# mlvlab/BLiM

Measured on AMD Instinct MI355X. Metric: candidate-pairs/sec (7B, 96+32 tok), higher is better.
Workload: dtype f16; 1 GPU; SYN v2t-VTG re-rank: Qwen2-7B dims (28 layers), seeded synthetic weights, 96 video + 32 text tokens per pair, top-16 text candidates per video query, 55 queries (880 pairs, 32560 packed tokens, 28160 label rows) per step per GPU; prefix_reuse=True, vtg_compensated=none, parallelism=query rows sharded over 1 GPU(s); RCCL all-gather of score rows at the end

## Files before the change

### blim_amd/csrc/attention.hip

```cpp
#include "attention.hpp"

#include <stdlib.h>

#include <type_traits>

#define HD 128
#define KT 32
#define QB 32

typedef __attribute__((ext_vector_type(4))) short s16x4;

template <int MAXC, bool SPLIT> struct attn_bound { static constexpr int value = MAXC <= (SPLIT ? 8 : 4) ? 512 : MAXC <= (SPLIT ? 16 : 8) ? 256 : 64; };
template <bool USE_TR, int MAXC, int DT, bool SPLIT = false, bool OUT_LO = SPLIT, bool PC = false>
__global__ __launch_bounds__((attn_bound<MAXC, SPLIT>::value)) void attn_kernel(const typename std::conditional<PC, AttnPcParams, AttnParams>::type p) {
    __shared__ __attribute__((aligned(16))) bf16_t k_lds[(SPLIT ? 2 : 1) * KT * HD];
    __shared__ __attribute__((aligned(16))) bf16_t v_lds[(SPLIT ? 2 : 1) * KT * HD];
    __shared__ uint32_t vis_lds[KT / 4];

    const int tid = threadIdx.x, nthreads = blockDim.x;
    const int lane = tid & 63;
    const int wave = tid >> 6;
    const int G = p.num_heads / p.num_kv_heads;
    const int ngrp = (int)gridDim.y / p.num_kv_heads;
    const int kh = blockIdx.y / ngrp, hg = blockIdx.y - kh * ngrp;
// ... 253 lines not shown
            if (hf == 0) {
                const int rl = (int)(tok & 255);
                p.out_mx[(int64_t)head * p.mx_stride + (tok >> 8) * 256 + ((rl >> 7) * 16 + (rl & 15)) * 8 + ((rl >> 4) & 7)] = (uint8_t)(e + 127);
            }
        }
        return;
    }
    if (q0 + qi < slen) {
        const float inv = l_run > 0.f ? 1.0f / l_run : 0.f;
        bf16_t* orow = p.out + (int64_t)(sstart + q0 + qi) * p.ldo + head * HD;
        if (p.lse_out && hf == 0) p.lse_out[(int64_t)(sstart + q0 + qi) * p.num_heads + head] = l_run > 0.f ? m_run * p.scale + __logf(l_run) : 1.0e30f;
#pragma unroll
        for (int db = 0; db < 4; ++db)
#pragma unroll
            for (int g = 0; g < 4; ++g) {
                const int d = 32 * db + 8 * g + 4 * hf;
                const float x0 = o[db][4 * g] * inv, x1 = o[db][4 * g + 1] * inv, x2 = o[db][4 * g + 2] * inv, x3 = o[db][4 * g + 3] * inv;
                *(uint2*)(orow + d) = make_uint2(pack2<DT>(x0, x1), pack2<DT>(x2, x3));
                if constexpr (OUT_LO)
                    *(uint2*)(orow + p.out_lo_off + d) = make_uint2(pack2<DT>(x0 - from16<DT>(to16<DT>(x0)), x1 - from16<DT>(to16<DT>(x1))),
                                                                    pack2<DT>(x2 - from16<DT>(to16<DT>(x2)), x3 - from16<DT>(to16<DT>(x3))));
            }
    }
}

static bool stages_tile(int maxc, const dim3& block, bool split) {
    if (maxc * (int)block.x >= (split ? 2048 : 1024)) return true;
    blim_set_error("attention: %d threads x %d staging chunks do not cover a tile's %d", (int)block.x, maxc, split ? 2048 : 1024);
    return false;
}

static int launch_attention_pc(const AttnPcParams& p, int G, hipStream_t stream) {
    const dim3 grid(p.n_blocks, p.num_kv_heads), block(64 * G);
    static const int g_split = getenv("BLIM_ATTN_HEAD_GROUPS") ? atoi(getenv("BLIM_ATTN_HEAD_GROUPS")) : 2;
#define ATTN_PC(MC, SP, OL, GRID, BLOCK)                                                                                           \
    do {                                                                                                                       \
        if (!stages_tile(MC, BLOCK, SP)) return BLIM_ERR_ARG;                                                                  \
        if (p.dtype == DT_F16) hipLaunchKernelGGL((attn_kernel<true, MC, DT_F16, SP, OL, true>), GRID, BLOCK, 0, stream, p);      \
        else hipLaunchKernelGGL((attn_kernel<true, MC, DT_BF16, SP, OL, true>), GRID, BLOCK, 0, stream, p);                   \
    } while (0)
    if (p.v_lo_off != 0) {
        if (p.out_lo_off) { if (G >= 7) ATTN_PC(5, true, true, grid, block); else ATTN_PC(4, true, true, grid, dim3(512)); }
        else { if (G >= 7) ATTN_PC(5, true, false, grid, block); else ATTN_PC(4, true, false, grid, dim3(512)); }
    } else if (p.out_lo_off != 0) {
        if (G >= 7 && g_split > 1) ATTN_PC(4, false, true, dim3(p.n_blocks, p.num_kv_heads * 2), dim3(64 * ((G + 1) / 2)));
        else if (G >= 5 && g_split > 1) ATTN_PC(8, false, true, dim3(p.n_blocks, p.num_kv_heads * 2), dim3(64 * ((G + 1) / 2)));
// ... 6 lines not shown
        else if (G >= 4) ATTN_PC(4, false, false, grid, block);
        else if (G >= 2) ATTN_PC(8, false, false, grid, block);
        else ATTN_PC(16, false, false, grid, block);
    }
#undef ATTN_PC
    hipError_t e = hipGetLastError();
    if (e != hipSuccess) { blim_set_error("attention launch failed: %s", hipGetErrorString(e)); return BLIM_ERR_HIP; }
    return BLIM_OK;
}

int launch_attention_cached(const AttnPcParams& p, hipStream_t stream) {
    ARG_CHECK(p.qkv && p.out && p.key_visible && p.seq_start && p.seq_len && p.pfx_start && p.pfx_len && p.blk_seq && p.blk_q0);
    ARG_CHECK(p.n_blocks > 0 && p.num_kv_heads > 0 && p.num_heads % p.num_kv_heads == 0);
    ARG_CHECK(p.ldq % 8 == 0 && p.ldo % 4 == 0);
    ARG_CHECK(p.pfx_cache && p.pfx_slot && p.pc_n_slots > 0 && p.pc_max_len > 0 && p.pc_ld % 8 == 0 && p.pc_lo_off % 8 == 0 && p.pc_slot_stride % 8 == 0 && p.pc_lo_off >= 0);
    ARG_CHECK((p.dtype == DT_F16 || p.dtype == DT_BF16) && p.v_lo_off >= 0 && p.out_lo_off >= 0 && p.v_lo_off % 8 == 0 && p.out_lo_off % 4 == 0);
    if (p.out8 || p.lse_out) { blim_set_error("attention: the prefix-cache forms write a 16-bit output and no lse"); return BLIM_ERR_ARG; }
    if (p.v_lo_off != 0 && p.pc_lo_off == 0) { blim_set_error("attention: a compensated call needs a prefix cache that holds lo parts"); return BLIM_ERR_ARG; }
    const int G = p.num_heads / p.num_kv_heads;
    if (G > 8) { blim_set_error("attention: %d query heads per kv head > 8 unsupported", G); return BLIM_ERR_ARG; }
    return launch_attention_pc(p, G, stream);
}

int launch_attention(const AttnParams& p, int use_tr_read, hipStream_t stream) {
    ARG_CHECK(p.qkv && p.out && p.key_visible && p.seq_start && p.seq_len && p.pfx_start && p.pfx_len && p.blk_seq && p.blk_q0);
    ARG_CHECK(p.n_blocks > 0 && p.num_kv_heads > 0 && p.num_heads % p.num_kv_heads == 0);
    ARG_CHECK(p.ldq % 8 == 0 && p.ldo % 4 == 0);
    const int G = p.num_heads / p.num_kv_heads;
    if (G > 8) { blim_set_error("attention: %d query heads per kv head > 8 unsupported", G); return BLIM_ERR_ARG; }
    const dim3 grid(p.n_blocks, p.num_kv_heads), block(64 * G);
    if (p.v_lo_off != 0 || p.out_lo_off != 0)
        ARG_CHECK((p.dtype == DT_F16 || p.dtype == DT_BF16) && p.v_lo_off >= 0 && p.out_lo_off >= 0 && p.v_lo_off % 8 == 0 && p.out_lo_off % 4 == 0 && !p.out8);
    if (p.v_lo_off != 0) {
#define ATTN_SPLIT(MC, BLOCK)                                                                                                       \
        do {                                                                                                                      \
            if (!stages_tile(MC, BLOCK, true)) return BLIM_ERR_ARG;                                                               \
            if (p.out_lo_off) {                                                                                                   \
                if (p.dtype == DT_F16) hipLaunchKernelGGL((attn_kernel<true, MC, DT_F16, true>), grid, BLOCK, 0, stream, p);       \
                else hipLaunchKernelGGL((attn_kernel<true, MC, DT_BF16, true>), grid, BLOCK, 0, stream, p);                    \
            } else {                                                                                                              \
                if (p.dtype == DT_F16) hipLaunchKernelGGL((attn_kernel<true, MC, DT_F16, true, false>), grid, BLOCK, 0, stream, p); \
                else hipLaunchKernelGGL((attn_kernel<true, MC, DT_BF16, true, false>), grid, BLOCK, 0, stream, p);              \
            }                                                                                                                     \
        } while (0)
        if (G >= 7) ATTN_SPLIT(5, block);
        else ATTN_SPLIT(4, dim3(512));
#undef ATTN_SPLIT
        hipError_t e2 = hipGetLastError();
        if (e2 != hipSuccess) { blim_set_error("attention launch failed: %s", hipGetErrorString(e2)); return BLIM_ERR_HIP; }
        return BLIM_OK;
// ... 2 lines not shown
    if (p.out_lo_off != 0) {
#define ATTN_LO(MC, GRID, BLOCK)                                                                                                   \
        do {                                                                                                                     \
            if (!stages_tile(MC, BLOCK, false)) return BLIM_ERR_ARG;                                                             \
            if (p.dtype == DT_F16) hipLaunchKernelGGL((attn_kernel<true, MC, DT_F16, false, true>), GRID, BLOCK, 0, stream, p);   \
            else hipLaunchKernelGGL((attn_kernel<true, MC, DT_BF16, false, true>), GRID, BLOCK, 0, stream, p);                \
        } while (0)
        if (G >= 7 && g_split > 1) ATTN_LO(4, dim3(p.n_blocks, p.num_kv_heads * 2), dim3(64 * ((G + 1) / 2)));
        else if (G >= 5 && g_split > 1) ATTN_LO(8, dim3(p.n_blocks, p.num_kv_heads * 2), dim3(64 * ((G + 1) / 2)));
        else if (G >= 4) ATTN_LO(4, grid, block);
        else if (G >= 2) ATTN_LO(8, grid, block);
        else ATTN_LO(16, grid, block);
#undef ATTN_LO
        hipError_t e3 = hipGetLastError();
        if (e3 != hipSuccess) { blim_set_error("attention launch failed: %s", hipGetErrorString(e3)); return BLIM_ERR_HIP; }
        return BLIM_OK;
    }
#define ATTN_LAUNCH(TR, MC)                                                                             \
    do {                                                                                            \
        if (!stages_tile(MC, block, false)) return BLIM_ERR_ARG;                                    \
        if (p.dtype == DT_F16) hipLaunchKernelGGL((attn_kernel<TR, MC, DT_F16>), grid, block, 0, stream, p); \
        else hipLaunchKernelGGL((attn_kernel<TR, MC, DT_BF16>), grid, block, 0, stream, p);                \
    } while (0)
    if (G >= 5 && g_split > 1 && use_tr_read && !p.out8) {
        const int hpg = (G + 1) / 2;
        const dim3 grid2(p.n_blocks, p.num_kv_heads * 2), block2(64 * hpg);
        if (!stages_tile(hpg >= 4 ? 4 : 8, block2, false)) return BLIM_ERR_ARG;
        if (hpg >= 4) {
            if (p.dtype == DT_F16) hipLaunchKernelGGL((attn_kernel<true, 4, DT_F16>), grid2, block2, 0, stream, p);
            else hipLaunchKernelGGL((attn_kernel<true, 4, DT_BF16>), grid2, block2, 0, stream, p);
        } else {
            if (p.dtype == DT_F16) hipLaunchKernelGGL((attn_kernel<true, 8, DT_F16>), grid2, block2, 0, stream, p);
            else hipLaunchKernelGGL((attn_kernel<true, 8, DT_BF16>), grid2, block2, 0, stream, p);
        }
    } else if (G >= 4) { if (use_tr_read) ATTN_LAUNCH(true, 4); else ATTN_LAUNCH(false, 4); }
    else if (G >= 2) { if (use_tr_read) ATTN_LAUNCH(true, 8); else ATTN_LAUNCH(false, 8); }
    else { if (use_tr_read) ATTN_LAUNCH(true, 16); else ATTN_LAUNCH(false, 16); }
#undef ATTN_LAUNCH
    hipError_t e = hipGetLastError();
    if (e != hipSuccess) { blim_set_error("attention launch failed: %s", hipGetErrorString(e)); return BLIM_ERR_HIP; }
    return BLIM_OK;
}
```

### blim_amd/csrc/attention.hpp

```cpp
#pragma once
#include "common.hpp"

struct AttnParams {
    int dtype;
    const bf16_t* qkv;
    int64_t ldq;
    int num_heads, num_kv_heads;
    const uint8_t* key_visible;
    const int32_t* seq_start;
    const int32_t* seq_len;
    const int32_t* pfx_start;
    const int32_t* pfx_len;
    const int32_t* blk_seq;
    const int32_t* blk_q0;
    const int32_t* own_start;
    int n_blocks;
    bf16_t* out;
    int64_t ldo;
    float scale;
    int64_t v_lo_off, out_lo_off;
    uint8_t* out8;
    int64_t ldo8;
    uint8_t* out_mx;
    int64_t mx_stride;
    float* lse_out;
};

int launch_attention(const AttnParams& p, int use_tr_read, hipStream_t stream);

struct AttnPcParams : AttnParams {
    const bf16_t* pfx_cache;
    const int32_t* pfx_slot;
    int64_t pc_slot_stride, pc_ld, pc_lo_off;
    int pc_n_slots, pc_max_len;
};
int launch_attention_cached(const AttnPcParams& p, hipStream_t stream);
```

### blim_amd/csrc/engine.hip

```cpp
#include <math.h>
#include <stdarg.h>
#include <stddef.h>
#include <stdio.h>
#include <stdlib.h>
#include <string.h>

#include <algorithm>
#include <map>
#include <string>
#include <vector>

#include "engine.hpp"

static thread_local char g_err[1024] = "";
void blim_set_error(const char* fmt, ...) {
    va_list ap;
    va_start(ap, fmt);
    vsnprintf(g_err, sizeof(g_err), fmt, ap);
    va_end(ap);
}
extern "C" const char* blim_last_error(void) { return g_err; }
extern "C" int blim_abi_version(void) { return BLIM_ABI_VERSION; }

static const char* kTimeClassNames[TC_COUNT] = {"gemm_qkv_rope", "attention", "gemm_o_resid", "gemm_gateup_swiglu", "gemm_down_resid",
// ... 837 lines not shown
            const blim_prefix_cache* pc = e->pc_fill;
            const int kvh = 2 * c.num_kv_heads * 128;
            TRY(launch_kv_capture(qkv, (int64_t)pf * e->qkv_n, (int64_t)c.num_heads * 128, (cA && pc->comp) ? e->qkv_n : 0, kvh, e->pc_cap_row, T,
                                  pc->kv + (int64_t)li * pc->max_len * pc->kv_w, pc->slot_stride, pc->kv_w, kvh, pc->max_len, pc->n_slots, s));
        }
        {
            SpanGuard g(e, s, TC_ATTN, 0);
            AttnParams a;
            a.dtype = c.compute_dtype;
            a.qkv = qkv; a.ldq = (int64_t)pf * e->qkv_n; a.num_heads = c.num_heads; a.num_kv_heads = c.num_kv_heads;
            a.key_visible = b->key_visible; a.seq_start = b->seq_start; a.seq_len = b->seq_len; a.pfx_start = b->pfx_start; a.pfx_len = b->pfx_len;
            a.blk_seq = b->blk_seq; a.blk_q0 = b->blk_q0; a.own_start = b->own_start; a.n_blocks = b->n_blocks; a.out = attn; a.ldo = (int64_t)pf * Hq; a.scale = 0.08838834764831845f;
            a.v_lo_off = cA ? e->qkv_n : 0; a.out_lo_off = cO ? Hq : 0;
            a.out8 = nullptr; a.ldo8 = 0; a.out_mx = nullptr; a.mx_stride = 0; a.lse_out = nullptr;
            if (o8 && e->f8_fuse) { a.out8 = a8; a.ldo8 = H; a.out_mx = (uint8_t*)e->attn_mx.p; a.mx_stride = Tp; }
            if (e->pc_read) {
                const blim_prefix_cache* pc = e->pc_read;
                AttnPcParams pa;
                static_cast<AttnParams&>(pa) = a;
                pa.pfx_cache = pc->kv + (int64_t)li * pc->max_len * pc->kv_w; pa.pfx_slot = e->pc_slot; pa.pc_slot_stride = pc->slot_stride; pa.pc_ld = pc->kv_w;
                pa.pc_lo_off = pc->comp ? 2 * c.num_kv_heads * 128 : 0; pa.pc_n_slots = pc->n_slots; pa.pc_max_len = pc->max_len;
                TRY(launch_attention_cached(pa, s));
            } else {
                TRY(launch_attention(a, e->attn_tr, s));
            }
            if (e->masked_query_zero) TRY(launch_zero_rows(attn, (int64_t)pf * Hq, b->key_visible, T, (int)(pf * Hq), s));
        }
        const bool fuse_o = o8 && e->f8_fuse;
        if (o8 && !fuse_o) { SpanGuard g(e, s, TC_QUANT, 0); TRY(launch_quant_rows(attn, H, T, H, c.compute_dtype, a8, sa, s)); }
        if (prune && li == c.num_layers - 1) {
            bf16_t* attn_live = act;
            float* rl = (float*)e->resid_live.p;
            {
                SpanGuard g0(e, s, TC_MISC, 0);
                TRY(launch_gather_rows(attn_live, attn, live_rows, n_live, (int64_t)pf * Hq * 2, T, 0u, s));
                if (G) TRY(adapter_u(e, attn_live, (int64_t)pf * Hq, cO ? Hq : 0, n_live, H, &e->AD[li].ad[3], nullptr, nullptr, s));
                TRY(launch_gather_rows(rl, resid, live_rows, n_live, (int64_t)H * 4, T, 0x7fc00000u, s));
            }
            const double tl = (double)n_live;
            { SpanGuard g(e, s, TC_GEMM_O, 2.0 * tl * Hq * H * (cO ? 2 : 1));
              GemmParams p = gp3(e, attn_live, Hq, G ? (const void*)e->AD[li].wo_aug : (const void*)l.wo, n_live, H, rl, H, 0, pf, cO, false); p.ldc = H; p.lo_off = 0;
              if (lo6 && cO) { p = gp(c.compute_dtype, attn_live, 2 * Hq, G ? (const void*)e->AD[li].wo_aug : (const void*)l.wo, n_live, H, (int)Hq, rl, H);
                         TRY(attach_lo6(p, attn_live, 2 * Hq, n_live, (int)Hq, G ? e->AD[li].wo_aug6 : l.wo6)); }
              TRY(launch_gemm(EPI_RESID, p, s)); }
            { SpanGuard g(e, s, TC_NORM, 0);
              TRY(launch_rmsnorm(rl, H, nullptr, n_live, H, l.norm2, c.rms_eps, xn, c.compute_dtype, nullptr, s, 0, pfm * H, (cG && !n2_tiles) ? xn + H : nullptr, true, n2_tiles ? (uint8_t*)e->a6.p : nullptr)); }
            { SpanGuard g(e, s, TC_GEMM_GATEUP, 4.0 * tl * H * I * (cG ? 2 : 1));
// ... 583 lines not shown
    ARG_CHECK(A_hilo && W && a6 && w6 && C && K % 128 == 0);
    hipStream_t s = (hipStream_t)stream;
    TRY(launch_f6_tiles((const bf16_t*)W, K, N, K, DT_F16, true, (uint8_t*)w6, s));
    TRY(launch_f6_tiles((const bf16_t*)A_hilo + K, 2 * (int64_t)K, M, K, DT_F16, false, (uint8_t*)a6, s));
    HIP_TRY(hipMemsetAsync(C, 0, (size_t)M * N * 4, s));
    GemmParams p = gp(DT_F16, A_hilo, 2 * (int64_t)K, W, M, N, K, C, N);
    p.A6 = (const uint8_t*)a6; p.W6 = (const uint8_t*)w6; p.K6 = K;
    return launch_gemm(EPI_RESID, p, s);
}
extern "C" int blim_quant_rows(const void* in16, int64_t ld, int64_t n_rows, int32_t K, int32_t dtype16, void* out8, float* scale, void* stream) {
    ARG_CHECK(dtype16 == BLIM_COMPUTE_BF16 || dtype16 == BLIM_COMPUTE_F16);
    return launch_quant_rows((const bf16_t*)in16, ld, n_rows, K, dtype16, (uint8_t*)out8, scale, (hipStream_t)stream);
}
extern "C" int blim_gemm_f8(const void* A8, int64_t lda, const float* a_scale, const void* W8, const float* w_scale, int32_t M, int32_t N, int32_t K,
                            void* C, int64_t ldc, void* stream) {
    GemmParams p = gp8(A8, lda, a_scale, W8, w_scale, M, N, K, C, ldc);
    return launch_gemm(EPI_BF16, p, (hipStream_t)stream);
}
extern "C" int blim_attention(const blim_attention_args* args, void* stream) {
    ARG_CHECK(args && args->struct_bytes >= (int64_t)offsetof(blim_attention_args, lse_out));
    blim_attention_args a;
    memset(&a, 0, sizeof a);
    memcpy(&a, args, (size_t)std::min<int64_t>(args->struct_bytes, (int64_t)sizeof a));
    const blim_batch* b = a.batch;
    ARG_CHECK(b && a.qkv && a.out);
    ARG_CHECK(b->n_tokens > 0 && b->n_seqs > 0 && b->n_blocks > 0);
    ARG_CHECK(b->key_visible && b->seq_start && b->seq_len && b->pfx_start && b->pfx_len && b->blk_seq && b->blk_q0);
    ARG_CHECK(a.dtype16 == BLIM_COMPUTE_BF16 || a.dtype16 == BLIM_COMPUTE_F16);
    ARG_CHECK(a.num_heads > 0 && a.num_kv_heads > 0 && a.num_heads % a.num_kv_heads == 0);
    if (a.num_heads / a.num_kv_heads > 8) { blim_set_error("attention: %d query heads per kv head > 8 unsupported", a.num_heads / a.num_kv_heads); return BLIM_ERR_ARG; }
    ARG_CHECK(a.ldq % 8 == 0 && a.ldo % 4 == 0 && a.v_lo_off >= 0 && a.out_lo_off >= 0 && a.v_lo_off % 8 == 0 && a.out_lo_off % 4 == 0);
    const int64_t qn = (int64_t)(a.num_heads + 2 * a.num_kv_heads) * 128, hn = (int64_t)a.num_heads * 128, cn = (int64_t)2 * a.num_kv_heads * 128;
    ARG_CHECK(a.ldq >= qn && a.ldo >= hn);
    if (a.v_lo_off && (a.v_lo_off < qn || a.v_lo_off + qn > a.ldq)) { blim_set_error("attention: the lo parts at v_lo_off overlap [q | k | v] or leave the row (ldq)"); return BLIM_ERR_ARG; }
    if (a.out_lo_off && (a.out_lo_off < hn || a.out_lo_off + hn > a.ldo)) { blim_set_error("attention: the lo output at out_lo_off overlaps the output or leaves the row (ldo)"); return BLIM_ERR_ARG; }
    if ((a.v_lo_off || a.out_lo_off) && !a.use_tr_read) { blim_set_error("attention: the compensated forms read V transposed (use_tr_read = 1)"); return BLIM_ERR_ARG; }
    if (a.out8) {
        ARG_CHECK(a.out_mx && a.dtype16 == BLIM_COMPUTE_F16 && a.ldo8 >= (int64_t)a.num_heads * 128 && a.ldo8 % 4 == 0 && a.mx_stride >= ((b->n_tokens + 255) / 256) * 256);
        if (a.v_lo_off || a.out_lo_off || a.lse_out) { blim_set_error("attention: the fused e4m3 output belongs to the plain form, without lse_out"); return BLIM_ERR_ARG; }
    }
    AttnPcParams p;
    memset(&p, 0, sizeof p);
    p.dtype = a.dtype16 == BLIM_COMPUTE_F16 ? DT_F16 : DT_BF16;
    p.qkv = (const bf16_t*)a.qkv; p.ldq = a.ldq; p.num_heads = a.num_heads; p.num_kv_heads = a.num_kv_heads;
    p.key_visible = b->key_visible; p.seq_start = b->seq_start; p.seq_len = b->seq_len; p.pfx_start = b->pfx_start; p.pfx_len = b->pfx_len;
    p.blk_seq = b->blk_seq; p.blk_q0 = b->blk_q0; p.own_start = b->own_start; p.n_blocks = b->n_blocks; p.out = (bf16_t*)a.out; p.ldo = a.ldo; p.scale = a.scale;
    p.v_lo_off = a.v_lo_off; p.out_lo_off = a.out_lo_off;
    p.out8 = (uint8_t*)a.out8; p.ldo8 = a.ldo8; p.out_mx = (uint8_t*)a.out_mx; p.mx_stride = a.mx_stride; p.lse_out = a.lse_out;
    if (!a.pfx_cache) return launch_attention(p, a.use_tr_read, (hipStream_t)stream);
    if (a.out8 || a.lse_out) { blim_set_error("attention: the prefix-cache forms write a 16-bit output and no lse"); return BLIM_ERR_ARG; }
    if (!a.use_tr_read) { blim_set_error("attention: the prefix-cache forms read V transposed (use_tr_read = 1)"); return BLIM_ERR_ARG; }
    if (a.v_lo_off != 0 && a.pc_lo_off == 0) { blim_set_error("attention: a compensated call needs a prefix cache that holds lo parts"); return BLIM_ERR_ARG; }
    ARG_CHECK(a.pfx_slot && a.pc_n_slots > 0 && a.pc_max_len > 0 && a.pc_ld % 8 == 0 && a.pc_lo_off % 8 == 0 && a.pc_slot_stride % 8 == 0 && a.pc_lo_off >= 0);
    ARG_CHECK(a.pc_ld >= cn && a.pc_slot_stride >= a.pc_max_len * a.pc_ld);
    if (a.pc_lo_off && (a.pc_lo_off < cn || a.pc_lo_off + cn > a.pc_ld)) { blim_set_error("attention: the cache's lo parts at pc_lo_off overlap [k | v] or leave the row (pc_ld)"); return BLIM_ERR_ARG; }
    p.pfx_cache = (const bf16_t*)a.pfx_cache; p.pfx_slot = a.pfx_slot; p.pc_slot_stride = a.pc_slot_stride; p.pc_ld = a.pc_ld; p.pc_lo_off = a.pc_lo_off;
    p.pc_n_slots = a.pc_n_slots; p.pc_max_len = a.pc_max_len;
    return launch_attention_cached(p, (hipStream_t)stream);
}

extern "C" int blim_gemm(const blim_gemm_args* args, void* stream) {
    ARG_CHECK(args && args->struct_bytes >= (int64_t)offsetof(blim_gemm_args, bias));
    blim_gemm_args a;
    memset(&a, 0, sizeof a);
    memcpy(&a, args, (size_t)std::min<int64_t>(args->struct_bytes, (int64_t)sizeof a));
    hipStream_t s = (hipStream_t)stream;
    ARG_CHECK(a.epi >= BLIM_EPI_BF16 && a.epi <= BLIM_EPI_LSE);
    ARG_CHECK(a.dtype == BLIM_COMPUTE_BF16 || a.dtype == BLIM_COMPUTE_F16 || a.dtype == BLIM_COMPUTE_F8);
    ARG_CHECK(a.A && a.W && a.M > 0 && a.N > 0 && a.K > 0 && a.lda > 0);
    const bool f8 = a.dtype == BLIM_COMPUTE_F8;
    const int64_t es = f8 ? 1 : 2;
    ARG_CHECK(a.K * es % 128 == 0 && a.lda * es % 16 == 0);
// ... 93 lines not shown
    return BLIM_OK;
}
extern "C" int blim_debug_read(blim_engine* e, const char* which, void* dst, int64_t bytes, void* stream) {
    ARG_CHECK(e && which && dst && bytes > 0);
    const DevBuf* b = nullptr;
    if (!strcmp(which, "resid")) b = &e->resid;
    else if (!strcmp(which, "xn")) b = &e->xn;
    else if (!strcmp(which, "qkv")) b = &e->qkv;
    else if (!strcmp(which, "attn")) b = &e->attn;
    else if (!strcmp(which, "act")) b = &e->act;
    else if (!strcmp(which, "act8")) b = &e->act8;
    else if (!strcmp(which, "act_mx")) b = &e->act_mx;
    if (!b || !b->p || (size_t)bytes > b->bytes) { blim_set_error("debug_read: no buffer '%s' of %lld bytes", which, (long long)bytes); return BLIM_ERR_ARG; }
    HIP_TRY(hipMemcpyAsync(dst, b->p, (size_t)bytes, hipMemcpyDeviceToDevice, (hipStream_t)stream));
    return BLIM_OK;
}
extern "C" int blim_debug_gemm_stamps(void* device_buf) {
    gemm_set_debug_stamps((unsigned long long*)device_buf);
    return BLIM_OK;
}
extern "C" int blim_set_option(blim_engine* e, const char* key, int32_t value) {
    ARG_CHECK(e && key);
    if (!strcmp(key, "attn_tr_read")) { e->attn_tr = value; return BLIM_OK; }
    if (!strcmp(key, "f8_mask")) { e->f8_mask = value & 31; return BLIM_OK; }
    if (!strcmp(key, "f8_fuse")) { e->f8_fuse = value != 0; return BLIM_OK; }
    if (!strcmp(key, "precise_embeds")) { e->precise_embeds = value != 0; return BLIM_OK; }
    if (!strcmp(key, "prune_last")) { e->prune_last = value != 0; return BLIM_OK; }
    if (!strcmp(key, "masked_query_zero")) {
        if (value && e->f8) { blim_set_error("option 'masked_query_zero' needs a 16-bit engine (the fp8 mode's attention output leaves the kernel quantised)"); return BLIM_ERR_ARG; }
        e->masked_query_zero = value != 0; return BLIM_OK;
    }
    if (!strcmp(key, "precise_lo6")) {
        if (value && e->f8) { blim_set_error("option 'precise_lo6' needs a 16-bit engine (fp16: the default; bf16: opt-in)"); return BLIM_ERR_ARG; }
        if (value && (e->c.hidden_size % 128 || e->c.intermediate_size % 128 || e->c.hidden_size > 20480 || e->c.intermediate_size > 20480)) {
            blim_set_error("option 'precise_lo6': hidden and intermediate sizes must be multiples of 128, at most 20480"); return BLIM_ERR_ARG; }
        if (value && e->aug && e->aug % 128) { blim_set_error("option 'precise_lo6': adapters were loaded with a %d-column K extension; set the option before loading adapters", e->aug); return BLIM_ERR_STATE; }
        e->lo6 = value != 0; return BLIM_OK;
    }
    if (!strcmp(key, "precise_mlp")) { e->precise_mlp = value != 0; return BLIM_OK; }
    if (!strcmp(key, "precise_layers")) {
        if (value && e->f8) { blim_set_error("option 'precise_layers' needs a 16-bit engine (fp16 or bf16)"); return BLIM_ERR_ARG; }
        e->layer_mask_on = value != 0; return BLIM_OK;
    }
    if (!strcmp(key, "precise_layer_bits")) {
        if (e->f8) { blim_set_error("option 'precise_layer_bits' needs a 16-bit engine (fp16 or bf16)"); return BLIM_ERR_ARG; }
        const int32_t layer = value >> 4;
// ... 13 lines not shown
```

### blim_amd/csrc/engine.hpp

```cpp
#pragma once
#include <map>
#include <set>
#include <string>
#include <vector>

#include "../../include/blim.h"
#include "adapters.hpp"
#include "attention.hpp"
#include "common.hpp"
#include "gemm.hpp"
#include "kernels.hpp"

#define TRY(expr)                 \
    do {                          \
        int _rc = (expr);         \
        if (_rc != BLIM_OK) return _rc; \
    } while (0)

enum TimeClass { TC_GEMM_QKV = 0, TC_ATTN, TC_GEMM_O, TC_GEMM_GATEUP, TC_GEMM_DOWN, TC_NORM, TC_LMHEAD_LSE, TC_GEMM_OTHER, TC_MISC, TC_QUANT, TC_COUNT };
struct TimedSpan { hipEvent_t a, b; int cls; double flops; };

struct DevBuf {
    void* p = nullptr;
    size_t bytes = 0;
// ... 36 lines not shown
    int hd = 128;
    int qkv_n = 0;
    std::vector<LayerW> L;
    bf16_t* embed = nullptr; bf16_t* lm_head = nullptr; bf16_t* visual_head = nullptr;
    float* final_norm = nullptr;
    bf16_t* mlp_w0[2] = {nullptr, nullptr}; float* mlp_b0[2] = {nullptr, nullptr};
    bf16_t* mlp_w2[2] = {nullptr, nullptr}; float* mlp_b2[2] = {nullptr, nullptr};
    float* rope_cos = nullptr; float* rope_sin = nullptr;
    bool f8 = false;
    bool f8_ready = false;
    int f8_mask = 31;
    uint8_t* lm_head8 = nullptr; float* s_lm = nullptr;
    std::map<std::string, bool> loaded;
    std::vector<void*> owned;
    DevBuf resid, xn, qkv, attn, act, hsel, lse_part, lab_logit, logprob, stage, proj_tmp, vh, tvg_logits, dense_idx;
    DevBuf rope_rows;
    DevBuf resid_live;
    bool prune_last = true;
    DevBuf x8, a8, act8, hsel8, rscale;
    DevBuf attn_mx;
    DevBuf act_mx;
    int f8_fuse = 1;
    int attn_tr = 1;
    bool precise = false;
    bool precise_mlp = true;
    bool layer_mask_on = false;
    std::vector<uint8_t> layer_bits;
    bool masked_query_zero = false;
    bool precise_embeds = false;
    bool timing = false;
    std::vector<TimedSpan> spans;
    int lora_r = 0; float lora_scale = 0.f; int aug = 0;
    std::vector<LayerAd> AD; AdapterW ad_lm, ad_mlp[2][2];
    uint16_t* lm_aug = nullptr; uint16_t* w0_aug[2] = {nullptr, nullptr}; uint16_t* w2_aug[2] = {nullptr, nullptr};
    bool aug_ready = false;
    bool lo6 = false, lo6_ready = false, lo6_fuse = true; int lo6_fuse_mask = 3;
    uint8_t* lm6 = nullptr;
    int lm6_k = 0;
    const void* lm6_src = nullptr;
    std::set<const void*> c6_dirty;
    DevBuf a6, a6b, h6;
    std::set<std::string> merged_pending;
    bool lora_merged = false;
    std::vector<void*> aug_owned;
    std::vector<void*> ad_owned;
    DevBuf feats_aug, hid_aug;
// ... 31 lines not shown
```

### blim_amd/engine.py

```python
from __future__ import annotations

import ctypes as C
import os
import re
from typing import Dict, Optional, Sequence

import numpy as np

from .synth import ModelDims, weight_shapes

_HERE = os.path.dirname(os.path.abspath(__file__))
LIB_PATH = os.environ.get("BLIM_LIB_PATH") or os.path.join(_HERE, "libblim_hip.so")
HEADER_PATH = os.path.join(os.path.dirname(_HERE), "include", "blim.h")

DTYPE_F32, DTYPE_BF16 = 0, 1
COMPUTE_DTYPES = {"bf16": 0, "f16": 1, "f8": 2}
DEFAULT_COMPUTE_DTYPE = os.environ.get("BLIM_DTYPE", "f16")


def torch_dtype_of(name: str):
    import torch
    return {"bf16": torch.bfloat16, "f16": torch.float16, "f8": torch.float16}[name]


# ... 1 lines not shown
    pass


class Config(C.Structure):
    _fields_ = [("vocab_size", C.c_int32), ("hidden_size", C.c_int32), ("intermediate_size", C.c_int32),
                ("num_layers", C.c_int32), ("num_heads", C.c_int32), ("num_kv_heads", C.c_int32),
                ("mm_hidden_size", C.c_int32), ("num_clips", C.c_int32), ("max_positions", C.c_int32),
                ("compute_dtype", C.c_int32), ("rms_eps", C.c_float), ("rope_theta", C.c_float)]


class Batch(C.Structure):
    _fields_ = [("n_tokens", C.c_int64), ("n_seqs", C.c_int32), ("n_blocks", C.c_int32),
                ("positions", C.c_void_p), ("key_visible", C.c_void_p), ("seq_start", C.c_void_p),
                ("seq_len", C.c_void_p), ("pfx_start", C.c_void_p), ("pfx_len", C.c_void_p),
                ("blk_seq", C.c_void_p), ("blk_q0", C.c_void_p), ("own_start", C.c_void_p)]


class AttentionArgs(C.Structure):
    _fields_ = [("struct_bytes", C.c_int64), ("batch", C.POINTER(Batch)), ("qkv", C.c_void_p), ("ldq", C.c_int64),
                ("num_heads", C.c_int32), ("num_kv_heads", C.c_int32), ("dtype16", C.c_int32), ("use_tr_read", C.c_int32),
                ("v_lo_off", C.c_int64), ("out_lo_off", C.c_int64), ("out", C.c_void_p), ("ldo", C.c_int64), ("scale", C.c_float),
                ("lse_out", C.c_void_p), ("out8", C.c_void_p), ("ldo8", C.c_int64), ("out_mx", C.c_void_p), ("mx_stride", C.c_int64),
                ("pfx_cache", C.c_void_p), ("pfx_slot", C.c_void_p), ("pc_slot_stride", C.c_int64), ("pc_ld", C.c_int64), ("pc_lo_off", C.c_int64),
                ("pc_n_slots", C.c_int32), ("pc_max_len", C.c_int32)]


class AttentionBwdArgs(C.Structure):
    _fields_ = [("struct_bytes", C.c_int64), ("qkv", C.c_void_p), ("ldq", C.c_int64), ("dout", C.c_void_p), ("ldo", C.c_int64), ("o16", C.c_void_p),
                ("ldo16", C.c_int64), ("lse", C.c_void_p), ("num_heads", C.c_int32), ("num_kv_heads", C.c_int32), ("dtype16", C.c_int32),
                ("key_visible", C.c_void_p), ("seq_start", C.c_void_p), ("seq_len", C.c_void_p), ("n_seqs", C.c_int32), ("max_len", C.c_int32),
                ("scale", C.c_float), ("workspace", C.c_void_p), ("workspace_bytes", C.c_int64), ("dqkv", C.c_void_p), ("n_tokens", C.c_int64)]


class GemmArgs(C.Structure):
    _fields_ = [("struct_bytes", C.c_int64), ("epi", C.c_int32), ("dtype", C.c_int32), ("A", C.c_void_p), ("lda", C.c_int64), ("W", C.c_void_p),
                ("M", C.c_int32), ("N", C.c_int32), ("K", C.c_int32), ("act", C.c_int32), ("C", C.c_void_p), ("ldc", C.c_int64), ("bias", C.c_void_p),
                ("resid_in", C.c_void_p), ("scale", C.c_float), ("w_wrap_k", C.c_int32), ("lo_off", C.c_int64), ("f16_saturate", C.c_int32),
                ("rope_cols", C.c_int32), ("rope_rows", C.c_void_p), ("rope_stride", C.c_int64), ("labels", C.c_void_p), ("lse_part", C.c_void_p),
                ("label_logit", C.c_void_p), ("row_scale", C.c_void_p), ("col_scale", C.c_void_p), ("a_mx", C.c_void_p), ("out8", C.c_void_p),
                ("out_mx", C.c_void_p), ("mx_stride", C.c_int64), ("A6", C.c_void_p), ("W6", C.c_void_p), ("K6", C.c_int32), ("f6_build", C.c_int32),
                ("out6", C.c_void_p), ("swiglu_act", C.c_void_p), ("swiglu_act_ld", C.c_int64), ("swiglu_gu", C.c_void_p), ("swiglu_ld", C.c_int64)]


EPILOGUES = {"bf16": 0, "f32": 1, "resid": 2, "qkv": 3, "swiglu": 4, "lse": 5}


def declared_symbols(header: str = HEADER_PATH) -> Sequence[str]:
# ... 524 lines not shown
    lib = load_library()
    M, K = a8.shape
    N = w8.shape[0]
    out = torch.empty((M, N), dtype=torch.float16, device=a8.device)
    _check(lib.blim_gemm_f8(_ptr(a8), K, _ptr(a_scale), _ptr(w8), _ptr(w_scale), M, N, K, _ptr(out), N, _stream()), "blim_gemm_f8")
    return out


def gemm_f16_lo6(a_hilo, w):
    import torch
    lib = load_library()
    M, K2 = a_hilo.shape
    N, K = w.shape
    assert K2 == 2 * K and a_hilo.dtype == torch.float16 and w.dtype == torch.float16 and a_hilo.is_contiguous() and w.is_contiguous()
    a6 = torch.empty(lib.blim_f6_tiles_bytes(M, K), dtype=torch.uint8, device=w.device)
    w6 = torch.empty(lib.blim_f6_tiles_bytes(N, K), dtype=torch.uint8, device=w.device)
    out = torch.empty((M, N), dtype=torch.float32, device=w.device)
    _check(lib.blim_gemm_f16_lo6(_ptr(a_hilo), _ptr(w), M, N, K, _ptr(a6), _ptr(w6), _ptr(out), _stream()), "blim_gemm_f16_lo6")
    return out, a6.view(-1, K // 128, 25600), w6.view(-1, K // 128, 25600)


def attention(qkv, batch: PackedBatch, num_heads: int, num_kv_heads: int, out, scale: float = 128 ** -0.5, use_tr_read: int = 1, v_lo_off: int = 0,
              out_lo_off: int = 0, lse_out=None, out8=None, out_mx=None, mx_stride: int = 0, pfx_cache=None, pfx_slot=None, pc_slot_stride: int = 0,
              pc_ld: int = 0, pc_lo_off: int = 0, pc_n_slots: int = 0, pc_max_len: int = 0):
    import torch
    lib = load_library()
    assert qkv.dim() == 2 and out.dim() == 2 and qkv.dtype == out.dtype and qkv.dtype in (torch.bfloat16, torch.float16)
    bs = batch.struct()
    a = AttentionArgs()
    a.struct_bytes = C.sizeof(AttentionArgs)
    a.batch = C.pointer(bs); a.qkv = _ptr(qkv); a.ldq = qkv.shape[1]; a.num_heads = num_heads; a.num_kv_heads = num_kv_heads
    a.dtype16 = COMPUTE_DTYPES["bf16" if qkv.dtype == torch.bfloat16 else "f16"]; a.use_tr_read = int(use_tr_read)
    a.v_lo_off = v_lo_off; a.out_lo_off = out_lo_off; a.out = _ptr(out); a.ldo = out.shape[1]; a.scale = scale
    a.lse_out = _ptr(lse_out); a.out8 = _ptr(out8); a.ldo8 = out8.shape[1] if out8 is not None else 0; a.out_mx = _ptr(out_mx); a.mx_stride = mx_stride
    a.pfx_cache = _ptr(pfx_cache); a.pfx_slot = _ptr(pfx_slot); a.pc_slot_stride = pc_slot_stride; a.pc_ld = pc_ld; a.pc_lo_off = pc_lo_off
    a.pc_n_slots = pc_n_slots; a.pc_max_len = pc_max_len
    _check(lib.blim_attention(C.byref(a), _stream()), "blim_attention")
    return out


def attention_bwd_workspace_bytes(n_tokens: int, n_seqs: int, num_heads: int, max_len: int) -> int:
    return int(load_library().blim_attention_bwd_workspace_bytes(n_tokens, n_seqs, num_heads, max_len))


def attention_bwd(qkv, dout, o16, lse, batch: PackedBatch, num_heads: int, num_kv_heads: int, max_len: int, dqkv, workspace, scale: float = 128 ** -0.5):
    import torch
    lib = load_library()
    assert qkv.dim() == 2 and dout.dim() == 2 and o16.dim() == 2 and dqkv.shape == qkv.shape and dqkv.dtype == torch.float32 and lse.dtype == torch.float32
    assert qkv.dtype == dout.dtype == o16.dtype and qkv.dtype in (torch.bfloat16, torch.float16) and workspace.dtype == torch.uint8
    a = AttentionBwdArgs()
    a.struct_bytes = C.sizeof(AttentionBwdArgs)
    a.qkv = _ptr(qkv); a.ldq = qkv.shape[1]; a.dout = _ptr(dout); a.ldo = dout.shape[1]; a.o16 = _ptr(o16); a.ldo16 = o16.shape[1]; a.lse = _ptr(lse)
    a.num_heads = num_heads; a.num_kv_heads = num_kv_heads; a.dtype16 = COMPUTE_DTYPES["bf16" if qkv.dtype == torch.bfloat16 else "f16"]
    a.key_visible = _ptr(batch.key_visible); a.seq_start = _ptr(batch.seq_start); a.seq_len = _ptr(batch.seq_len); a.n_seqs = batch.n_seqs; a.max_len = max_len
    a.scale = scale; a.workspace = _ptr(workspace); a.workspace_bytes = workspace.numel(); a.dqkv = _ptr(dqkv); a.n_tokens = qkv.shape[0]
    _check(lib.blim_attention_bwd(C.byref(a), _stream()), "blim_attention_bwd")
    return dqkv


# ... 57 lines not shown
```

### include/blim.h

```cpp
#ifndef BLIM_H_
#define BLIM_H_
#include <stdint.h>
#ifdef __cplusplus
extern "C" {
#endif

#define BLIM_ABI_VERSION 9
#define BLIM_ERR_ARG (-1)
#define BLIM_ERR_HIP (-2)
#define BLIM_ERR_STATE (-3)
#define BLIM_ERR_NOMEM (-4)

#define BLIM_DTYPE_F32 0
#define BLIM_DTYPE_BF16 1

#define BLIM_COMPUTE_BF16 0
#define BLIM_COMPUTE_F16 1
#define BLIM_COMPUTE_F8 2

typedef struct blim_engine blim_engine;

typedef struct blim_config {
    int32_t vocab_size, hidden_size, intermediate_size, num_layers, num_heads, num_kv_heads;
    int32_t mm_hidden_size;
// ... 96 lines not shown
int blim_gemm_f8(const void* A8, int64_t lda, const float* a_scale, const void* W8, const float* w_scale, int32_t M, int32_t N, int32_t K,
                 void* C, int64_t ldc, void* stream);
typedef struct blim_attention_args {
    int64_t struct_bytes;
    const blim_batch* batch;
    const void* qkv;
    int64_t ldq;
    int32_t num_heads, num_kv_heads;
    int32_t dtype16;
    int32_t use_tr_read;
    int64_t v_lo_off, out_lo_off;
    void* out;
    int64_t ldo;
    float scale;
    float* lse_out;
    void* out8;
    int64_t ldo8;
    void* out_mx;
    int64_t mx_stride;
    const void* pfx_cache;
    const int32_t* pfx_slot;
    int64_t pc_slot_stride, pc_ld, pc_lo_off;
    int32_t pc_n_slots, pc_max_len;
} blim_attention_args;
int blim_attention(const blim_attention_args* args, void* stream);

typedef struct blim_attention_bwd_args {
    int64_t struct_bytes;
    const void* qkv;
    int64_t ldq;
    const void* dout;
    int64_t ldo;
    const void* o16;
    int64_t ldo16;
    const float* lse;
    int32_t num_heads, num_kv_heads;
    int32_t dtype16;
    const uint8_t* key_visible;
    const int32_t* seq_start;
    const int32_t* seq_len;
    int32_t n_seqs, max_len;
    float scale;
    void* workspace;
    int64_t workspace_bytes;
    float* dqkv;
    int64_t n_tokens;
// ... 129 lines not shown
```

Baseline: 2673 pairs/s.

## Add grouped persistent attention kernel keeping shared prefix K/V resident in LDS

Adds a new attention kernel in which each workgroup walks a contiguous chunk of query blocks instead of one block. Prefix (video) K/V tiles of up to four tiles stay resident in LDS and are reused across consecutive blocks that share the same prefix. The next block's first tile and Q are prefetched during the last tile of the current block. The grid is sized to roughly two workgroups per CU. This targets redundant prefix K/V reloads and per-block launch and prologue overhead, at the cost of much more LDS per workgroup, less parallelism, and possible load imbalance.

```diff
diff --git a/blim_amd/csrc/attention.hip b/blim_amd/csrc/attention.hip
--- a/blim_amd/csrc/attention.hip
+++ b/blim_amd/csrc/attention.hip
@@ -299,6 +299,274 @@
                                                                     pack2<DT>(x2 - from16<DT>(to16<DT>(x2)), x3 - from16<DT>(to16<DT>(x3))));
             }
     }
+}
+
+#define ATTN_RES_TILES 4
+template <int DT>
+__global__ __launch_bounds__(512) void attn_grouped_kernel(const AttnParams p) {
+    constexpr int MAXC = 4;
+    __shared__ __attribute__((aligned(16))) bf16_t k_lds[(ATTN_RES_TILES + 1) * KT * HD];
+    __shared__ __attribute__((aligned(16))) bf16_t v_lds[(ATTN_RES_TILES + 1) * KT * HD];
+
+    const int tid = threadIdx.x, nthreads = blockDim.x;
+    const int lane = tid & 63;
+    const int wave = tid >> 6;
+    const int G = p.num_heads / p.num_kv_heads;
+    const int ngrp = (int)gridDim.y / p.num_kv_heads;
+    const int kh = blockIdx.y / ngrp, hg = blockIdx.y - kh * ngrp;
+    const int hpg = (G + ngrp - 1) / ngrp;
+    const int wave_head = hg * hpg + wave;
+    const bool worker = wave < hpg && wave_head < G;
+    const int head = kh * G + (worker ? wave_head : 0);
+    const int qi = lane & 31, hf = lane >> 5;
+    const int koff = p.num_heads * HD + kh * HD;
+    const int voff = (p.num_heads + p.num_kv_heads) * HD + kh * HD;
+    const float NEG = -1.0e30f;
+    const float c_log2 = p.scale * 1.4426950408889634f;
+    const int blk0 = (int)((int64_t)blockIdx.x * p.n_blocks / gridDim.x), blk1 = (int)((int64_t)(blockIdx.x + 1) * p.n_blocks / gridDim.x);
+
+    struct Blk { int q0, sstart, slen, pstart, plen; };
+    auto read_blk = [&](int blk) __attribute__((always_inline)) {
+        Blk b;
+        const int s = p.blk_seq[blk];
+        b.q0 = p.blk_q0[blk]; b.sstart = p.seq_start[s]; b.slen = p.seq_len[s]; b.plen = p.pfx_len[s];
+        b.pstart = b.plen > 0 ? p.pfx_start[s] : 0;
+        return b;
+    };
+    auto resident = [&](const Blk& b) __attribute__((always_inline)) { return b.plen > 0 && b.plen <= ATTN_RES_TILES * KT; };
+    auto load_q = [&](const Blk& b, bf16x8 (&q)[8], int& qstart) __attribute__((always_inline)) {
+        const int qtok = b.sstart + min(b.q0 + qi, b.slen - 1);
+        qstart = p.own_start ? p.own_start[qtok] : 0;
+        const bf16_t* qrow = p.qkv + (int64_t)qtok * p.ldq + head * HD + 8 * hf;
+#pragma unroll
+        for (int ks = 0; ks < 8; ++ks) q[ks] = *(const bf16x8*)(qrow + 16 * ks);
+    };
+
+    uint4 st[MAXC];
+    uint8_t st_vis = 0;
+#pragma unroll
+    for (int i = 0; i < MAXC; ++i) st[i] = make_uint4(0, 0, 0, 0);
+    auto load_into = [&](uint4 (&r)[MAXC], uint8_t& vis, int base_tok, int k0, int seg_len) __attribute__((always_inline)) {
+#pragma unroll
+        for (int i = 0; i < MAXC; ++i) {
+            const int idx = tid + i * nthreads;
+            if (idx < 1024) {
+                const int isv = idx >> 9, row = (idx >> 4) & 31, ch = idx & 15;
+                const int kk = min(k0 + row, seg_len - 1);
+                r[i] = *(const uint4*)(p.qkv + (int64_t)(base_tok + kk) * p.ldq + (isv ? voff : koff) + 8 * ch);
+            }
+        }
+        if (lane < KT) {
+            const int kk = k0 + lane;
+            vis = (kk < seg_len) ? p.key_visible[base_tok + kk] : (uint8_t)0;
+        }
+    };
+    auto store_from = [&](const uint4 (&r)[MAXC], uint8_t vis, int slot) __attribute__((always_inline)) {
+#pragma unroll
+        for (int i = 0; i < MAXC; ++i) {
+            const int idx = tid + i * nthreads;
+            if (idx < 1024) {
+                const int isv = idx >> 9, row = (idx >> 4) & 31, ch = idx & 15;
+                if (isv) *(uint4*)(v_lds + slot * KT * HD + row * HD + 8 * (ch ^ ((row & 3) << 2))) = r[i];
+                else *(uint4*)(k_lds + slot * KT * HD + row * HD + 8 * (ch ^ (row & 15))) = r[i];
+            }
+        }
+        return (uint32_t)__builtin_amdgcn_ballot_w64(lane < KT && vis != 0);
+    };
+    auto load_tile = [&](int base_tok, int k0, int seg_len) __attribute__((always_inline)) { load_into(st, st_vis, base_tok, k0, seg_len); };
+    auto store_tile = [&](int slot) __attribute__((always_inline)) { return store_from(st, st_vis, slot); };
+    auto load_first = [&](const Blk& b) __attribute__((always_inline)) {
+        if (b.plen > 0 && !resident(b)) load_tile(b.pstart, 0, b.plen);
+        else load_tile(b.sstart, 0, b.slen);
+    };
+
+    Blk cur = read_blk(blk0);
+    bf16x8 qf[8];
+    int qstart, qstart_n = 0;
+    load_q(cur, qf, qstart);
+    load_first(cur);
+    __builtin_amdgcn_s_waitcnt(0x0F70);
+
+    int r_pstart = -1, r_plen = 0;
+    uint32_t r_vis[ATTN_RES_TILES] = {0, 0, 0, 0};
+
+    for (int blk = blk0; blk < blk1; ++blk) {
+        const bool has_next = blk + 1 < blk1;
+        const Blk nxt = has_next ? read_blk(blk + 1) : cur;
+        const int q0 = cur.q0, sstart = cur.sstart, slen = cur.slen, pstart = cur.pstart, plen = cur.plen;
+        const int n_ptiles = (plen + KT - 1) / KT;
+        const int own_keys = min(q0 + QB, slen);
+        const int n_tiles = n_ptiles + (own_keys + KT - 1) / KT;
+        const bool res = resident(cur);
+        const int first_staged = res ? n_ptiles : 0;
+#if defined(ATTN_ABLATE) && ATTN_ABLATE == 1
+        const bool stage = blk == blk0;
+#else
+        const bool stage = true;
+#endif
+
+        uint32_t cur_vis = 0xFFFFFFFFu;
+        if (stage) {
+            if (blk > blk0) __syncthreads();
+            cur_vis = store_tile(ATTN_RES_TILES);
+            if (res && (pstart != r_pstart || plen != r_plen)) {
+                static_assert(ATTN_RES_TILES == 4, "the staging below names four register sets");
+                uint4 ps0[MAXC], ps1[MAXC], ps2[MAXC], ps3[MAXC];
+                uint8_t pv0 = 0, pv1 = 0, pv2 = 0, pv3 = 0;
+#pragma unroll
+                for (int i = 0; i < MAXC; ++i) ps0[i] = ps1[i] = ps2[i] = ps3[i] = make_uint4(0, 0, 0, 0);
+                load_into(ps0, pv0, pstart, 0, plen);
+                if (n_ptiles > 1) load_into(ps1, pv1, pstart, KT, plen);
+                if (n_ptiles > 2) load_into(ps2, pv2, pstart, 2 * KT, plen);
+                if (n_ptiles > 3) load_into(ps3, pv3, pstart, 3 * KT, plen);
+                r_vis[0] = store_from(ps0, pv0, 0);
+                if (n_ptiles > 1) r_vis[1] = store_from(ps1, pv1, 1);
+                if (n_ptiles > 2) r_vis[2] = store_from(ps2, pv2, 2);
+                if (n_ptiles > 3) r_vis[3] = store_from(ps3, pv3, 3);
+                r_pstart = pstart; r_plen = plen;
+            }
+            __syncthreads();
+        }
+
+        f32x16 o[4];
+#pragma unroll
+        for (int i = 0; i < 4; ++i)
+#pragma unroll
+            for (int r = 0; r < 16; ++r) o[i][r] = 0.f;
+        float m_run = NEG, l_run = 0.f;
+
+        for (int t = 0; t < n_tiles; ++t) {
+            const bool causal = t >= n_ptiles;
+            const int k0 = (causal ? t - n_ptiles : t) * KT;
+            int slot = ATTN_RES_TILES;
+            uint32_t vmask;
+            if (t < first_staged) {
+                slot = t;
+                vmask = t == 0 ? r_vis[0] : t == 1 ? r_vis[1] : t == 2 ? r_vis[2] : r_vis[3];
+            } else if (stage) {
+                if (t > first_staged) {
+                    __syncthreads();
+                    cur_vis = store_tile(ATTN_RES_TILES);
+                    __syncthreads();
+                }
+                if (t + 1 < n_tiles) {
+                    if (t + 1 < n_ptiles) load_tile(pstart, (t + 1) * KT, plen);
+                    else load_tile(sstart, (t + 1 - n_ptiles) * KT, slen);
+                }
+                vmask = cur_vis;
+            } else vmask = cur_vis;
+            const bool prefetch = t == n_tiles - 1 && has_next;
+            if (prefetch && stage) load_first(nxt);
+#if defined(ATTN_ABLATE) && ATTN_ABLATE == 2
+            if (prefetch) load_q(nxt, qf, qstart_n);
+            continue;
+#endif
+            if (!worker) { if (prefetch) load_q(nxt, qf, qstart_n); continue; }
+
+            const bf16_t* kt = k_lds + slot * KT * HD;
+            const bf16_t* vt = v_lds + slot * KT * HD;
+            f32x16 sacc;
+#pragma unroll
+            for (int r = 0; r < 16; ++r) sacc[r] = 0.f;
+            {
+                const int key = lane & 31;
+#pragma unroll
+                for (int ks = 0; ks < 8; ++ks) {
+                    const bf16x8 kf = *(const bf16x8*)(kt + key * HD + 8 * ((2 * ks + hf) ^ (key & 15)));
+                    sacc = mfma32<DT>(kf, qf[ks], sacc);
+                }
+            }
+            if (prefetch) load_q(nxt, qf, qstart_n);
+            float pv[16];
+            const bool vis_all = vmask == 0xFFFFFFFFu;
+            if (!vis_all || (causal && (k0 + KT - 1 > q0 || p.own_start != nullptr))) {
+#pragma unroll
+                for (int g = 0; g < 4; ++g) {
+#pragma unroll
+                    for (int j = 0; j < 4; ++j) {
+                        const int r = 4 * g + j;
+                        const int kk = k0 + 8 * g + 4 * hf + j;
+                        const bool ok = (((vmask >> (8 * g + 4 * hf + j)) & 1u) != 0) & (!causal | ((kk <= q0 + qi) & (kk >= qstart)));
+                        sacc[r] = ok ? sacc[r] : NEG;
+                    }
+                }
+            }
+            float tmax = NEG;
+#pragma unroll
+            for (int r = 0; r < 16; ++r) tmax = fmaxf(tmax, sacc[r]);
+            tmax = xhalf_max(tmax);
+            float m_new = m_run;
+            const bool move = tmax * c_log2 > m_run * c_log2 + 8.0f;
+            if (__builtin_amdgcn_ballot_w64(move) != 0) {
+                m_new = move ? fmaxf(m_run, tmax) : m_run;
+                const float alpha = __builtin_amdgcn_exp2f((m_run - m_new) * c_log2);
+                l_run *= alpha;
+#pragma unroll
+                for (int i = 0; i < 4; ++i)
+#pragma unroll
+                    for (int r = 0; r < 16; ++r) o[i][r] *= alpha;
+            }
+            const float mc = m_new > 0.5f * NEG ? m_new * c_log2 : 0.f;
+            float rsum = 0.f;
+#pragma unroll
+            for (int r = 0; r < 16; ++r) {
+                const float e = __builtin_amdgcn_exp2f(fmaf(sacc[r], c_log2, -mc));
+                pv[r] = e;
+                rsum += e;
+            }
+            l_run += xhalf_sum(rsum);
+            m_run = m_new;
+
+            bf16x8 pf[2];
+#pragma unroll
+            for (int s2 = 0; s2 < 2; ++s2) {
+                uint32_t w[4];
+#pragma unroll
+                for (int j = 0; j < 4; ++j) w[j] = pack2<DT>(pv[8 * s2 + 2 * j], pv[8 * s2 + 2 * j + 1]);
+                pf[s2] = __builtin_bit_cast(bf16x8, make_uint4(w[0], w[1], w[2], w[3]));
+            }
+#pragma unroll
+            for (int db = 0; db < 4; ++db) {
+#pragma unroll
+                for (int s2 = 0; s2 < 2; ++s2) {
+                    const int i16 = lane & 15, g16 = (lane >> 4) & 1;
+                    const int dcol = 32 * db + 16 * g16 + 4 * (i16 & 3);
+                    const int ch = dcol >> 3, within = dcol & 7;
+                    const int kr0 = 16 * s2 + 4 * hf + (i16 >> 2);
+                    const int kr1 = kr0 + 8;
+                    const s16x4 lo = __builtin_amdgcn_ds_read_tr16_b64_v4i16(
+                        (__attribute__((address_space(3))) s16x4*)(vt + kr0 * HD + 8 * (ch ^ ((kr0 & 3) << 2)) + within));
+                    const s16x4 hi = __builtin_amdgcn_ds_read_tr16_b64_v4i16(
+                        (__attribute__((address_space(3))) s16x4*)(vt + kr1 * HD + 8 * (ch ^ ((kr1 & 3) << 2)) + within));
+                    const bf16x8 vf = (bf16x8){lo[0], lo[1], lo[2], lo[3], hi[0], hi[1], hi[2], hi[3]};
+                    o[db] = mfma32<DT>(vf, pf[s2], o[db]);
+                }
+            }
+        }
+
+        if (worker && q0 + qi < slen) {
+            const float inv = l_run > 0.f ? 1.0f / l_run : 0.f;
+            bf16_t* orow = p.out + (int64_t)(sstart + q0 + qi) * p.ldo + head * HD;
+#pragma unroll
+            for (int db = 0; db < 4; ++db)
+#pragma unroll
+                for (int g = 0; g < 4; ++g) {
+                    const int d = 32 * db + 8 * g + 4 * hf;
+                    *(uint2*)(orow + d) = make_uint2(pack2<DT>(o[db][4 * g] * inv, o[db][4 * g + 1] * inv), pack2<DT>(o[db][4 * g + 2] * inv, o[db][4 * g + 3] * inv));
+                }
+        }
+        cur = nxt;
+        qstart = qstart_n;
+    }
+}
+
+static int attn_resident_workgroups() {
+    static const int cus = [] {
+        int dev = 0, n = 0;
+        if (hipGetDevice(&dev) != hipSuccess || hipDeviceGetAttribute(&n, hipDeviceAttributeMultiprocessorCount, dev) != hipSuccess || n <= 0) n = 256;
+        return n;
+    }();
+    return 2 * cus;
 }
 
 static bool stages_tile(int maxc, const dim3& block, bool split) {
@@ -351,10 +619,11 @@
     return launch_attention_pc(p, G, stream);
 }
 
-int launch_attention(const AttnParams& p, int use_tr_read, hipStream_t stream) {
+int launch_attention(const AttnParams& p, int use_tr_read, hipStream_t stream, int group_blocks) {
     ARG_CHECK(p.qkv && p.out && p.key_visible && p.seq_start && p.seq_len && p.pfx_start && p.pfx_len && p.blk_seq && p.blk_q0);
     ARG_CHECK(p.n_blocks > 0 && p.num_kv_heads > 0 && p.num_heads % p.num_kv_heads == 0);
     ARG_CHECK(p.ldq % 8 == 0 && p.ldo % 4 == 0);
+    ARG_CHECK(group_blocks >= -1 && group_blocks <= ATTN_GROUP_MAX);
     const int G = p.num_heads / p.num_kv_heads;
     if (G > 8) { blim_set_error("attention: %d query heads per kv head > 8 unsupported", G); return BLIM_ERR_ARG; }
     const dim3 grid(p.n_blocks, p.num_kv_heads), block(64 * G);
@@ -403,7 +672,20 @@
         if (p.dtype == DT_F16) hipLaunchKernelGGL((attn_kernel<TR, MC, DT_F16>), grid, block, 0, stream, p); \
         else hipLaunchKernelGGL((attn_kernel<TR, MC, DT_BF16>), grid, block, 0, stream, p);                \
     } while (0)
-    if (G >= 5 && g_split > 1 && use_tr_read && !p.out8) {
+    int nb = group_blocks >= 0 ? group_blocks : p.n_blocks >= ATTN_GROUP_MIN_BLOCKS ? ATTN_GROUP_DEFAULT : 0;
+    if (nb > 0 && G >= 4 && use_tr_read && !p.out8 && !p.lse_out) {
+        const bool two = G >= 5 && g_split > 1;
+        const int waves = max(4, two ? (G + 1) / 2 : G);
+        const int gy = p.num_kv_heads * (two ? 2 : 1);
+        const int slots = attn_resident_workgroups(), per_round = slots / gy;
+        if (group_blocks < 0) nb = min(nb, max(1, (int)((int64_t)p.n_blocks * gy / slots)));
+        int nx = (p.n_blocks + nb - 1) / nb;
+        if (per_round > 0 && nx > per_round && nx <= 4 * per_round) nx = min(p.n_blocks, (nx + per_round / 2) / per_round * per_round);
+        const dim3 gridg(nx, gy), blockg(64 * waves);
+        if (!stages_tile(4, blockg, false)) return BLIM_ERR_ARG;
+        if (p.dtype == DT_F16) hipLaunchKernelGGL((attn_grouped_kernel<DT_F16>), gridg, blockg, 0, stream, p);
+        else hipLaunchKernelGGL((attn_grouped_kernel<DT_BF16>), gridg, blockg, 0, stream, p);
+    } else if (G >= 5 && g_split > 1 && use_tr_read && !p.out8) {
         const int hpg = (G + 1) / 2;
         const dim3 grid2(p.n_blocks, p.num_kv_heads * 2), block2(64 * hpg);
         if (!stages_tile(hpg >= 4 ? 4 : 8, block2, false)) return BLIM_ERR_ARG;
diff --git a/blim_amd/csrc/attention.hpp b/blim_amd/csrc/attention.hpp
--- a/blim_amd/csrc/attention.hpp
+++ b/blim_amd/csrc/attention.hpp
@@ -26,7 +26,10 @@
     float* lse_out;
 };
 
-int launch_attention(const AttnParams& p, int use_tr_read, hipStream_t stream);
+#define ATTN_GROUP_DEFAULT 8
+#define ATTN_GROUP_MIN_BLOCKS 2
+#define ATTN_GROUP_MAX 1024
+int launch_attention(const AttnParams& p, int use_tr_read, hipStream_t stream, int group_blocks = -1);
 
 struct AttnPcParams : AttnParams {
     const bf16_t* pfx_cache;
diff --git a/blim_amd/csrc/engine.hip b/blim_amd/csrc/engine.hip
--- a/blim_amd/csrc/engine.hip
+++ b/blim_amd/csrc/engine.hip
@@ -883,7 +883,7 @@
                 pa.pc_lo_off = pc->comp ? 2 * c.num_kv_heads * 128 : 0; pa.pc_n_slots = pc->n_slots; pa.pc_max_len = pc->max_len;
                 TRY(launch_attention_cached(pa, s));
             } else {
-                TRY(launch_attention(a, e->attn_tr, s));
+                TRY(launch_attention(a, e->attn_tr, s, e->attn_group));
             }
             if (e->masked_query_zero) TRY(launch_zero_rows(attn, (int64_t)pf * Hq, b->key_visible, T, (int)(pf * Hq), s));
         }
@@ -1513,6 +1513,8 @@
     blim_attention_args a;
     memset(&a, 0, sizeof a);
     memcpy(&a, args, (size_t)std::min<int64_t>(args->struct_bytes, (int64_t)sizeof a));
+    if (args->struct_bytes < (int64_t)(offsetof(blim_attention_args, group_blocks) + sizeof a.group_blocks)) a.group_blocks = -1;
+    if (a.group_blocks < -1 || a.group_blocks > ATTN_GROUP_MAX) { blim_set_error("attention: group_blocks is 0, a chunk size up to %d, or -1 (got %d)", ATTN_GROUP_MAX, (int)a.group_blocks); return BLIM_ERR_ARG; }
     const blim_batch* b = a.batch;
     ARG_CHECK(b && a.qkv && a.out);
     ARG_CHECK(b->n_tokens > 0 && b->n_seqs > 0 && b->n_blocks > 0);
@@ -1538,7 +1540,7 @@
     p.blk_seq = b->blk_seq; p.blk_q0 = b->blk_q0; p.own_start = b->own_start; p.n_blocks = b->n_blocks; p.out = (bf16_t*)a.out; p.ldo = a.ldo; p.scale = a.scale;
     p.v_lo_off = a.v_lo_off; p.out_lo_off = a.out_lo_off;
     p.out8 = (uint8_t*)a.out8; p.ldo8 = a.ldo8; p.out_mx = (uint8_t*)a.out_mx; p.mx_stride = a.mx_stride; p.lse_out = a.lse_out;
-    if (!a.pfx_cache) return launch_attention(p, a.use_tr_read, (hipStream_t)stream);
+    if (!a.pfx_cache) return launch_attention(p, a.use_tr_read, (hipStream_t)stream, a.group_blocks);
     if (a.out8 || a.lse_out) { blim_set_error("attention: the prefix-cache forms write a 16-bit output and no lse"); return BLIM_ERR_ARG; }
     if (!a.use_tr_read) { blim_set_error("attention: the prefix-cache forms read V transposed (use_tr_read = 1)"); return BLIM_ERR_ARG; }
     if (a.v_lo_off != 0 && a.pc_lo_off == 0) { blim_set_error("attention: a compensated call needs a prefix cache that holds lo parts"); return BLIM_ERR_ARG; }
@@ -1678,6 +1680,10 @@
 extern "C" int blim_set_option(blim_engine* e, const char* key, int32_t value) {
     ARG_CHECK(e && key);
     if (!strcmp(key, "attn_tr_read")) { e->attn_tr = value; return BLIM_OK; }
+    if (!strcmp(key, "attn_group")) {
+        if (value < -1 || value > ATTN_GROUP_MAX) { blim_set_error("option 'attn_group': 0 (per-block kernel), a chunk size up to %d, or -1 (default); got %d", ATTN_GROUP_MAX, (int)value); return BLIM_ERR_ARG; }
+        e->attn_group = value; return BLIM_OK;
+    }
     if (!strcmp(key, "f8_mask")) { e->f8_mask = value & 31; return BLIM_OK; }
     if (!strcmp(key, "f8_fuse")) { e->f8_fuse = value != 0; return BLIM_OK; }
     if (!strcmp(key, "precise_embeds")) { e->precise_embeds = value != 0; return BLIM_OK; }
diff --git a/blim_amd/csrc/engine.hpp b/blim_amd/csrc/engine.hpp
--- a/blim_amd/csrc/engine.hpp
+++ b/blim_amd/csrc/engine.hpp
@@ -82,6 +82,7 @@
     DevBuf act_mx;
     int f8_fuse = 1;
     int attn_tr = 1;
+    int attn_group = -1;
     bool precise = false;
     bool precise_mlp = true;
     bool layer_mask_on = false;
diff --git a/blim_amd/engine.py b/blim_amd/engine.py
--- a/blim_amd/engine.py
+++ b/blim_amd/engine.py
@@ -47,7 +47,7 @@
                 ("v_lo_off", C.c_int64), ("out_lo_off", C.c_int64), ("out", C.c_void_p), ("ldo", C.c_int64), ("scale", C.c_float),
                 ("lse_out", C.c_void_p), ("out8", C.c_void_p), ("ldo8", C.c_int64), ("out_mx", C.c_void_p), ("mx_stride", C.c_int64),
                 ("pfx_cache", C.c_void_p), ("pfx_slot", C.c_void_p), ("pc_slot_stride", C.c_int64), ("pc_ld", C.c_int64), ("pc_lo_off", C.c_int64),
-                ("pc_n_slots", C.c_int32), ("pc_max_len", C.c_int32)]
+                ("pc_n_slots", C.c_int32), ("pc_max_len", C.c_int32), ("group_blocks", C.c_int32)]
 
 
 class AttentionBwdArgs(C.Structure):
@@ -618,7 +618,7 @@
 
 def attention(qkv, batch: PackedBatch, num_heads: int, num_kv_heads: int, out, scale: float = 128 ** -0.5, use_tr_read: int = 1, v_lo_off: int = 0,
               out_lo_off: int = 0, lse_out=None, out8=None, out_mx=None, mx_stride: int = 0, pfx_cache=None, pfx_slot=None, pc_slot_stride: int = 0,
-              pc_ld: int = 0, pc_lo_off: int = 0, pc_n_slots: int = 0, pc_max_len: int = 0):
+              pc_ld: int = 0, pc_lo_off: int = 0, pc_n_slots: int = 0, pc_max_len: int = 0, group_blocks: int = -1):
     import torch
     lib = load_library()
     assert qkv.dim() == 2 and out.dim() == 2 and qkv.dtype == out.dtype and qkv.dtype in (torch.bfloat16, torch.float16)
@@ -630,7 +630,7 @@
     a.v_lo_off = v_lo_off; a.out_lo_off = out_lo_off; a.out = _ptr(out); a.ldo = out.shape[1]; a.scale = scale
     a.lse_out = _ptr(lse_out); a.out8 = _ptr(out8); a.ldo8 = out8.shape[1] if out8 is not None else 0; a.out_mx = _ptr(out_mx); a.mx_stride = mx_stride
     a.pfx_cache = _ptr(pfx_cache); a.pfx_slot = _ptr(pfx_slot); a.pc_slot_stride = pc_slot_stride; a.pc_ld = pc_ld; a.pc_lo_off = pc_lo_off
-    a.pc_n_slots = pc_n_slots; a.pc_max_len = pc_max_len
+    a.pc_n_slots = pc_n_slots; a.pc_max_len = pc_max_len; a.group_blocks = group_blocks
     _check(lib.blim_attention(C.byref(a), _stream()), "blim_attention")
     return out
 
diff --git a/include/blim.h b/include/blim.h
--- a/include/blim.h
+++ b/include/blim.h
@@ -142,6 +142,7 @@
     const int32_t* pfx_slot;
     int64_t pc_slot_stride, pc_ld, pc_lo_off;
     int32_t pc_n_slots, pc_max_len;
+    int32_t group_blocks;
 } blim_attention_args;
 int blim_attention(const blim_attention_args* args, void* stream);
 
```

After: 2675 pairs/s, median of 3. No clear change (+0.1%).
